# rssalessio/TZDDPC

Hardware: AMD Instinct MI355X
Metric: MPC steps/sec (batched trajectories), double-integrator N=20 (higher is better)
Workload: dtype f64

## Files before the change

### tzddpc_amd/csrc/tz_ipm.hip.h

```cpp
#pragma once

#define TZ_MINWAVES 4
#define TZ_RLEV_CARRY_MAX 2
#define TZ_RLEV_GATE 1e6
#define TZ_SEED_VIOL_MAX 0.1

struct TzEll { int L, VL; const TzEllEnt* ent; const int* seg; const double* val; const unsigned short* idx; };
typedef __attribute__((address_space(1))) const char* tz_gptr;
typedef __attribute__((address_space(1))) const tz_d2* tz_gd2ptr;
__device__ inline double tz_ell_walk(const char* base_, unsigned lo, int L, unsigned stride, const double* in) {
  double a0 = 0.0, a1 = 0.0;
  const char* b = reinterpret_cast<const char*>(in);
  tz_gptr base = (tz_gptr)base_;
  int e = 0;
  for (; e + 3 < L; e += 4) {
    tz_gptr q0 = base, q1 = base + stride, q2 = base + 2 * (size_t)stride, q3 = base + 3 * (size_t)stride;
    asm volatile("" : "+s"(q0), "+s"(q1), "+s"(q2), "+s"(q3));
    const tz_d2 r0 = *(tz_gd2ptr)(q0 + lo), r1 = *(tz_gd2ptr)(q1 + lo), r2 = *(tz_gd2ptr)(q2 + lo), r3 = *(tz_gd2ptr)(q3 + lo);
    base += 4 * (size_t)stride;
    a0 += r0.x * *reinterpret_cast<const double*>(b + tz_ell_off(r0.y));
    a1 += r1.x * *reinterpret_cast<const double*>(b + tz_ell_off(r1.y));
    a0 += r2.x * *reinterpret_cast<const double*>(b + tz_ell_off(r2.y));
    a1 += r3.x * *reinterpret_cast<const double*>(b + tz_ell_off(r3.y));
  }
// ... 418 lines not shown
    }
    if (pacc) { unsigned long long t1 = __builtin_amdgcn_s_memtime(); pacc[hh == 0 ? PH_GRAM_RED : PH_GRAM_RMW] += t1 - tq0; tq0 = t1; }
    if (hh == 0) __syncthreads();
    if (pacc && hh == 0) { unsigned long long t1 = __builtin_amdgcn_s_memtime(); pacc[PH_GRAM_BAR] += t1 - tq0; tq0 = t1; }
  }
}

__device__ inline void tz_form_H_ksplit(const IpmParams& p, double* Hq, const double* Pq, const double* wv, const int* sm, unsigned long long* pacc) {
  const int wave = __builtin_amdgcn_readfirstlane(threadIdx.x >> 6);
  const int g = wave >> 1, h = wave & 1;
  if (p.Tz > 7) { if (g == 0) tz_gram_rows<0, 7>(p, Hq, Pq, wv, sm, h, pacc); else tz_gram_rows<7, 10>(p, Hq, Pq, wv, sm, h, pacc); }
  else          { if (g == 0) tz_gram_rows<0, 5>(p, Hq, Pq, wv, sm, h, pacc); else tz_gram_rows<5, 7>(p, Hq, Pq, wv, sm, h, pacc); }
}

__device__ inline void tz_gram(const IpmParams& p, double* Hq, const double* Pq, const double* wv, const int* kl, unsigned long long* pacc = nullptr) {
  if (p.ksplit) tz_form_H_ksplit(p, Hq, Pq, wv, kl, pacc);
  else tz_form_H(p, Hq, wv, kl);
}

__device__ inline void tz_sqrt_rsqrt(double d, double& sq, double& rs) {
  double y = __builtin_amdgcn_rsq(d);
  double g = d * y, h = 0.5 * y;
  double r = __builtin_fma(-h, g, 0.5);
  g = __builtin_fma(g, r, g); h = __builtin_fma(h, r, h);
  const double e = __builtin_fma(-g, g, d);
  g = __builtin_fma(e, h, g);
  double inv = h + h;
  const double e2 = __builtin_fma(-g, inv, 1.0);
  inv = __builtin_fma(e2, inv, inv);
  sq = g; rs = inv;
}

__device__ inline double tz_recip(double x) {
  double y = __builtin_amdgcn_rcp(x);
  y = __builtin_fma(__builtin_fma(-x, y, 1.0), y, y);
  y = __builtin_fma(__builtin_fma(-x, y, 1.0), y, y);
  return y;
}

template <int JJ>
__device__ inline double tz_quad_bcast(double v) {
  const unsigned long long u = __builtin_bit_cast(unsigned long long, v);
  constexpr int ctrl = JJ * 0x55;
  const unsigned lo = (unsigned)__builtin_amdgcn_mov_dpp((int)(unsigned)u, ctrl, 0xf, 0xf, true);
  const unsigned hi = (unsigned)__builtin_amdgcn_mov_dpp((int)(unsigned)(u >> 32), ctrl, 0xf, 0xf, true);
  return __builtin_bit_cast(double, ((unsigned long long)hi << 32) | lo);
}

__device__ inline void tz_factor_col(int Tz, double* Hq, double* dinv, int* flag, int pp, int tid, int nthr) {
  const int dbase = (tz_qprefix(pp) + (pp >> 2)) * TZ_QSTR + 4 * (pp & 3);
  const double a00 = Hq[dbase], a10 = Hq[dbase + TZ_QROW], a11 = Hq[dbase + TZ_QROW + 1];
  const double a20 = Hq[dbase + 2 * TZ_QROW], a21 = Hq[dbase + 2 * TZ_QROW + 1], a22 = Hq[dbase + 2 * TZ_QROW + 2];
  const double a30 = Hq[dbase + 3 * TZ_QROW], a31 = Hq[dbase + 3 * TZ_QROW + 1], a32 = Hq[dbase + 3 * TZ_QROW + 2], a33 = Hq[dbase + 3 * TZ_QROW + 3];
  bool ok = true;
  double l00, i00, l11, i11, l22, i22, l33, i33;
  ok = ok && (a00 > 0.0);
  tz_sqrt_rsqrt(fmax(a00, 1e-300), l00, i00);
  const double l10 = a10 * i00, l20 = a20 * i00, l30 = a30 * i00;
  const double d1 = a11 - l10 * l10; ok = ok && (d1 > 0.0);
  tz_sqrt_rsqrt(fmax(d1, 1e-300), l11, i11);
  const double l21 = (a21 - l20 * l10) * i11, l31 = (a31 - l30 * l10) * i11;
  const double d2 = a22 - l20 * l20 - l21 * l21; ok = ok && (d2 > 0.0);
  tz_sqrt_rsqrt(fmax(d2, 1e-300), l22, i22);
  const double l32 = (a32 - l30 * l20 - l31 * l21) * i22;
  const double d3 = a33 - l30 * l30 - l31 * l31 - l32 * l32; ok = ok && (d3 > 0.0);
  tz_sqrt_rsqrt(fmax(d3, 1e-300), l33, i33);
  (void)l00; (void)l11; (void)l22; (void)l33;
  {
    const double m10 = -l10 * i00 * i11;
    const double m21 = -l21 * i11 * i22;
    const double m32 = -l32 * i22 * i33;
    const double m20 = -(l20 * i00 + l21 * m10) * i22;
    const double m31 = -(l31 * i11 + l32 * m21) * i33;
    const double m30 = -(l30 * i00 + l31 * m10 + l32 * m20) * i33;
    if (tid == 0 && !ok) *flag = 1;
    if (tid == 0) {
      double* m = dinv + pp * 16;
      m[0] = i00;
      m[4] = m10; m[5] = i11;
      m[8] = m20; m[9] = m21; m[10] = i22;
      m[12] = m30; m[13] = m31; m[14] = m32; m[15] = i33;
    }
  }
  for (int t = tid; t < 4 * (Tz - pp - 1); t += nthr) {
    const int I = pp + 1 + (t >> 2), i = t & 3;
    const int base = (tz_qprefix(I) + (pp >> 2)) * TZ_QSTR + TZ_QROW * i + 4 * (pp & 3);
    const double b0 = Hq[base], b1 = Hq[base + 1], b2 = Hq[base + 2], b3 = Hq[base + 3];
    const double x0 = b0 * i00;
    const double x1 = (b1 - x0 * l10) * i11;
    const double x2 = (b2 - x0 * l20 - x1 * l21) * i22;
    const double x3 = (b3 - x0 * l30 - x1 * l31 - x2 * l32) * i33;
    Hq[base] = x0; Hq[base + 1] = x1; Hq[base + 2] = x2; Hq[base + 3] = x3;
  }
}

__device__ inline void tz_wave_sync() {
  __builtin_amdgcn_fence(__ATOMIC_RELEASE, "wavefront");
  __builtin_amdgcn_wave_barrier();
  __builtin_amdgcn_fence(__ATOMIC_ACQUIRE, "wavefront");
}
__device__ inline bool tz_spin_until(const int* f, int target) {
  for (int guard = 0; guard < (1 << 20); ++guard) {
    const int v = __builtin_amdgcn_readfirstlane(__hip_atomic_load(f, __ATOMIC_ACQUIRE, __HIP_MEMORY_SCOPE_WORKGROUP));
    if (v >= target) return true;
    __builtin_amdgcn_s_sleep(1);
  }
  return false;
}

__device__ inline void tz_cholesky_wave(const IpmParams& p, double* Hq, double* dinv, int* flag, int* prog = nullptr) {
  const int Tz = p.Tz;
  const int lane = tz_tid() & 63;
  const int k = lane >> 4, blk = (lane >> 2) & 3, ij = lane & 3;
  for (int pp = 0; pp < Tz; ++pp) {
    if (pp > 0) {
      const int pq = pp >> 2, po = 4 * (pp & 3);
      const double* pb = Hq + tz_qprefix(pp) * TZ_QSTR + TZ_QROW * ij + k;
      for (int g = 0; pp + 4 * g < Tz; g += 2) {
        const int Ia = pp + 4 * g + blk, Ib = Ia + 4;
        const bool va = Ia < Tz, vb = Ib < Tz;
        const int qa = tz_qprefix(va ? Ia : pp), qb = tz_qprefix(vb ? Ib : pp);
        const double* pa = Hq + qa * TZ_QSTR + TZ_QROW * ij + k;
        const double* pa2 = Hq + qb * TZ_QSTR + TZ_QROW * ij + k;
        double* pc = Hq + (qa + pq) * TZ_QSTR + TZ_QROW * k + po + ij;
        double* pc2 = Hq + (qb + pq) * TZ_QSTR + TZ_QROW * k + po + ij;
        double a0 = *pc, a1 = 0.0, c0 = vb ? *pc2 : 0.0, c1 = 0.0;
        int off = 0, k2 = 0;
        for (; k2 + 1 < pp; k2 += 2) {
          const int off1 = off + 4 + (((k2 & 3) == 3) ? TZ_QSTR - 16 : 0);
          const double nb0 = -pb[off], nb1 = -pb[off1];
          const double x0 = pa[off], x1 = pa[off1], y0 = pa2[off], y1 = pa2[off1];
          a0 = __builtin_amdgcn_mfma_f64_4x4x4f64(x0, nb0, a0, 0, 0, 0);
          c0 = __builtin_amdgcn_mfma_f64_4x4x4f64(y0, nb0, c0, 0, 0, 0);
          a1 = __builtin_amdgcn_mfma_f64_4x4x4f64(x1, nb1, a1, 0, 0, 0);
          c1 = __builtin_amdgcn_mfma_f64_4x4x4f64(y1, nb1, c1, 0, 0, 0);
          off = off1 + 4 + ((((k2 + 1) & 3) == 3) ? TZ_QSTR - 16 : 0);
        }
        if (k2 < pp) {
          const double nb0 = -pb[off];
          a0 = __builtin_amdgcn_mfma_f64_4x4x4f64(pa[off], nb0, a0, 0, 0, 0);
          c0 = __builtin_amdgcn_mfma_f64_4x4x4f64(pa2[off], nb0, c0, 0, 0, 0);
        }
        if (va) *pc = a0 + a1;
        if (vb) *pc2 = c0 + c1;
      }
      tz_wave_sync();
    }
    tz_factor_col(Tz, Hq, dinv, flag, pp, lane, 64);
    tz_wave_sync();
    if (prog && lane == 0) __hip_atomic_store(prog, pp + 1, __ATOMIC_RELEASE, __HIP_MEMORY_SCOPE_WORKGROUP);
  }
}

__device__ inline void tz_chol_solve_wave(const IpmParams& p, const double* Hq, const double* dinv, const double* rhs, double* out, bool bwd_only = false) {
  const int tt = tz_tid();
  if (tt >= 64) return;
  __builtin_amdgcn_s_setprio(TZ_PRIO_SOLVE);
  const int Tz = p.Tz, nzp = p.nzp;
  const int t = tt, jq = t & 3, tq = t >> 2;
  double rv = (t < nzp) ? rhs[t] : 0.0;
  const int rowbase = tz_qprefix(tq < Tz ? tq : 0) * TZ_QSTR + TZ_QROW * jq;
  auto fwd_load = [&](int I, double (&mm)[4], double (&ll)[4]) {
    const int Ic = I < Tz ? I : Tz - 1;
    const double* m = dinv + Ic * 16 + 4 * jq;
    const int base = rowbase + (Ic >> 2) * TZ_QSTR + 4 * (Ic & 3);
    const bool below = tq > Ic && tq < Tz;
#pragma unroll
    for (int k = 0; k < 4; ++k) { mm[k] = m[k]; ll[k] = below ? Hq[base + k] : 0.0; }
  };
  double mA[4], lA[4], mB[4], lB[4];
  auto fwd_step = [&](int I, const double (&mm)[4], const double (&ll)[4]) {
    const double a0 = tz_quad_bcast<0>(rv), a1 = tz_quad_bcast<1>(rv), a2 = tz_quad_bcast<2>(rv), a3 = tz_quad_bcast<3>(rv);
    const double yc = (mm[0] * a0 + mm[1] * a1) + (mm[2] * a2 + mm[3] * a3);
    const double y0 = tz_readlane(yc, 4 * I), y1 = tz_readlane(yc, 4 * I + 1), y2 = tz_readlane(yc, 4 * I + 2), y3 = tz_readlane(yc, 4 * I + 3);
    rv = (tq == I) ? yc : rv - ((ll[0] * y0 + ll[1] * y1) + (ll[2] * y2 + ll[3] * y3));
  };
  if (!bwd_only) {
  fwd_load(0, mA, lA);
  for (int I = 0; I < Tz; I += 2) {
    fwd_load(I + 1, mB, lB);
    fwd_step(I, mA, lA);
    fwd_load(I + 2, mA, lA);
    if (I + 1 < Tz) fwd_step(I + 1, mB, lB);
  }
  }
  const int colbase = (t >> 4) * TZ_QSTR + 4 * ((t >> 2) & 3) + (t & 3);
  auto bwd_load = [&](int I, double (&mm)[4], double (&ll)[4]) {
    const int Ic = I >= 0 ? I : 0;
    const double* m = dinv + Ic * 16 + jq;
    const int base = tz_qprefix(Ic) * TZ_QSTR + colbase;
    const bool above = tq < Ic;
#pragma unroll
    for (int k = 0; k < 4; ++k) { mm[k] = m[4 * k]; ll[k] = above ? Hq[base + k * TZ_QROW] : 0.0; }
  };
  bwd_load(Tz - 1, mA, lA);
  for (int I = Tz - 1; I >= 0; I -= 2) {
    bwd_load(I - 1, mB, lB);
    fwd_step(I, mA, lA);
    bwd_load(I - 2, mA, lA);
    if (I - 1 >= 0) fwd_step(I - 1, mB, lB);
  }
  if (t < nzp) out[t] = rv;
  __builtin_amdgcn_s_setprio(0);
}

__device__ inline bool tz_fwd_trailing(const IpmParams& p, const double* Hq, const double* dinv, double rv, const int* prog, double* yout) {
  const int Tz = p.Tz, nzp = p.nzp;
  const int t = tz_tid() & 63, jq = t & 3, tq = t >> 2;
  const int rowbase = tz_qprefix(tq < Tz ? tq : 0) * TZ_QSTR + TZ_QROW * jq;
  bool ok = true;
  for (int I = 0; I < Tz; ++I) {
    if (!tz_spin_until(prog, I + 1)) { ok = false; break; }
    const double* m = dinv + I * 16 + 4 * jq;
    const int base = rowbase + (I >> 2) * TZ_QSTR + 4 * (I & 3);
    const bool below = tq > I && tq < Tz;
    double mm[4], ll[4];
#pragma unroll
    for (int k = 0; k < 4; ++k) { mm[k] = m[k]; ll[k] = below ? Hq[base + k] : 0.0; }
    const double a0 = tz_quad_bcast<0>(rv), a1 = tz_quad_bcast<1>(rv), a2 = tz_quad_bcast<2>(rv), a3 = tz_quad_bcast<3>(rv);
    const double yc = (mm[0] * a0 + mm[1] * a1) + (mm[2] * a2 + mm[3] * a3);
    const double y0 = tz_readlane(yc, 4 * I), y1 = tz_readlane(yc, 4 * I + 1), y2 = tz_readlane(yc, 4 * I + 2), y3 = tz_readlane(yc, 4 * I + 3);
    rv = (tq == I) ? yc : rv - ((ll[0] * y0 + ll[1] * y1) + (ll[2] * y2 + ll[3] * y3));
  }
  if (t < nzp) yout[t] = rv;
  return ok;
}

#include "tz_tt.hip.h"
#define TZ_TT_NST 4
#define TZ_TT_AFTER_CHOL(p, H, dinv) do { tz_tt_block_inverse(p, H, dinv); __syncthreads(); } while (0)
#define TZ_TT_SOLVE(p, H, dinv, rhs, ybuf, out) tz_chol_solve_blk(p, H, rhs, ybuf, out)


typedef __attribute__((address_space(4))) const IpmParams* TzKargPtr;

template <int MAXR, int NCG, int MINW = TZ_MINWAVES>
__global__ __launch_bounds__(TZ_THREADS, MINW) void tz_ipm_kernel(IpmParams p) {
#if TZ_PROFILE
  const bool PROF = p.prof != nullptr && blockIdx.x == 0;
#else
  constexpr bool PROF = false;
#endif
  unsigned long long tprev = 0, tstart = 0;
  unsigned long long acc_ph[PH_COUNT] = {};
#define TZ_STAMP(ph) do { if (PROF) { unsigned long long _t = __builtin_amdgcn_s_memtime(); acc_ph[ph] += _t - tprev; tprev = _t; } } while (0)
  if (PROF) { tprev = __builtin_amdgcn_s_memtime(); tstart = tprev; }
  extern __shared__ double lds[];
  const int b = blockIdx.x;
  int t = threadIdx.x;
#define TZ_FRESH_T() asm volatile("" : "+v"(t))
#define TZ_COLS(c, lim) if (const int c = t; c < (lim))
  const bool wave0 = __builtin_amdgcn_readfirstlane(threadIdx.x >> 6) == 0;
  const bool wave1 = __builtin_amdgcn_readfirstlane(threadIdx.x >> 6) == 1;
  const int nz = p.nz, mi = p.mi, nzp = p.nzp, mip = p.mip;
  const FuseParams& F0 = p.F;
  const bool fused = F0.on != 0;
  if (!fused && p.prestatus[b] != 0) {
    if (t == 0) { p.status[b] = 3; p.iters[b] = 0; if (p.status_copy) p.status_copy[b] = 3; }
    TZ_COLS(c, nz) p.x[(size_t)b * nz + c] = 0.0;
    for (int r = t; r < mi; r += TZ_THREADS) { p.s[(size_t)b * mi + r] = 1.0; p.lam[(size_t)b * mi + r] = 0.0; }
    return;
  }
  constexpr bool TT = (NCG >= 2);
  const size_t hsize = TT ? (size_t)p.ntile * p.TS : (size_t)p.nquads * TZ_QSTR;
  double* Hq = lds;
  double* dinv = Hq + hsize;
  double* dfac = dinv + p.Tz * 16;
  double* xv = dfac + (TT ? 16 : 0);
  double* dxv = xv + nzp;
  double* rdv = dxv + nzp;
  double* r1v = rdv + nzp;
  double* qv = r1v + nzp;
  double* tmpz = qv + nzp;
  double* part = tmpz + nzp;
  double* part2 = part + 4 * nzp;
  double* vin = part2 + 4 * nzp;
  double* red = vin + mip + 4;
  int* flag = (int*)(red + 32);
  int* kl = (int*)(red + 34);
  double* thl = red + 34 + (p.nklist + 1) / 2;
  double* stl = thl + p.F.ntheta;
  double* pl = stl + 4 * TZ_NMAX;
  double* tbl = pl + p.nell;
  double* Pq = tbl + p.ntube;
  constexpr bool PARK = (MINW == 4);
  double* hL = Pq + (p.ksplit ? hsize : 0);
  double* gL = hL + mip;

  double s_[MAXR], l_[MAXR], h_[MAXR], gx_[MAXR];
#define TZ_H(k, r) (PARK ? hL[r] : h_[k])
#define TZ_GX(k, r) (PARK ? gL[r] : gx_[k])
#define TZ_SET_H(k, r, v) do { if (PARK) hL[r] = (v); else h_[k] = (v); } while (0)
#define TZ_ADD_GX(k, r, v) do { if (PARK) gL[r] += (v); else gx_[k] += (v); } while (0)
#define TZ_ROWS(k, r) _Pragma("unroll") for (int k = 0; k < MAXR; ++k) if (const int r = t + TZ_THREADS * k; r < mi)
  int rseg_[MAXR];
#pragma unroll
  for (int k = 0; k < MAXR; ++k) { const int r = t + TZ_THREADS * k; rseg_[k] = (r < mi) ? p.eg.seg[r] : 0; }
  const int ccol = (nzp <= 64 && t >= 64) ? (t < 128 ? t - 64 : nz) : t;
  const int cseg = (ccol < nz) ? p.et.seg[ccol] : 0;

  if (TT) { (void)kl; (void)Pq; }
  else if (p.ksplit) {
    for (int i = t; i <= ((p.Kc + 3) >> 2); i += TZ_THREADS) kl[i] = p.smask[i];
    for (int e = t; e < p.nquads * 64; e += TZ_THREADS) {
      const int qd = e >> 6;
      int I = 0;
      while (tz_qprefix(I + 1) <= qd) ++I;
      const int r = 4 * I + ((e >> 4) & 3), c = 4 * (4 * (qd - tz_qprefix(I)) + ((e >> 2) & 3)) + (e & 3);
      double v = (c < nzp) ? p.P[(size_t)r * nzp + c] : 0.0;
      if (r == c) v = (r < nz) ? v + p.reg : 1.0;
      Pq[qd * TZ_QSTR + TZ_QROW * ((e >> 4) & 3) + (e & 15)] = v;
    }
  }
  else for (int i = t; i < p.nklist; i += TZ_THREADS) kl[i] = p.klist[i];
  if (fused) {
    const int n = F0.fin.n, m = F0.fin.m, nv = F0.fin.N * m;
    const int n1 = (F0.tube.pmax + 1) * n * n, n2 = n1 + (F0.tube.pmax > 0 ? F0.tube.pmax : 1) * (n + m) * n;
    for (int i = t; i < n2; i += TZ_THREADS) tbl[i] = (i < n1) ? F0.tube.CKpow[i] : F0.tube.T[i - n1];
    double* ec = tbl + n2;
    const double* plA = F0.plant.A + (size_t)b * F0.plant.A_stride;
    const double* plB = F0.plant.Bm + (size_t)b * F0.plant.B_stride;
    for (int i = t; i < n * n; i += TZ_THREADS) { ec[i] = plA[i]; ec[2 * n * m + n * n + n + i] = F0.fin.R2[i]; ec[2 * n * m + 2 * n * n + n + i] = F0.fin.Phi[(size_t)n * n + i]; }
    for (int i = t; i < n * m; i += TZ_THREADS) { ec[n * n + i] = plB[i]; ec[n * n + n * m + i] = F0.plant.K[i]; }
    for (int i = t; i < n; i += TZ_THREADS) ec[n * n + 2 * n * m + i] = F0.fin.r1[i];
    for (int i = t; i < n * nv; i += TZ_THREADS) ec[3 * n * n + 2 * n * m + n + i] = F0.fin.Gam[(size_t)n * nv + i];
    for (int i = t; i < nv; i += TZ_THREADS) ec[3 * n * n + 2 * n * m + n + n * nv + i] = F0.fin.Dz[i];
    int* pwl = (int*)(ec + 3 * n * n + 2 * n * m + n + n * nv + nv);
    for (int i = t; i < F0.fin.N; i += TZ_THREADS) pwl[i] = F0.tube.power[i];
  }
  if (fused && t < F0.fin.n) {
    stl[t] = F0.plant.x[(size_t)b * F0.fin.n + t];
    stl[F0.fin.n + t] = F0.plant.xbar[(size_t)b * F0.fin.n + t];
    stl[2 * F0.fin.n + t] = F0.plant.e[(size_t)b * F0.fin.n + t];
  }
#pragma unroll
  for (int k = 0; k < MAXR; ++k) { s_[k] = 1.0; l_[k] = 0.0; h_[k] = 0.0; gx_[k] = 0.0; }
  TZ_COLS(c, nzp) xv[c] = 0.0;
  for (int c = t; c < p.Tz * 16; c += TZ_THREADS) dinv[c] = 0.0;
  for (int r = t; r < mip + 4; r += TZ_THREADS) vin[r] = 0.0;
  __syncthreads();

  const int nsteps = fused ? F0.nsteps : 1;
  if (fused && F0.sticky_fresh != 0 && t == 0 && F0.plant.sticky) F0.plant.sticky[b] = 0;
  int was_shifted = (p.warm != 0 && (p.shift_policy >= 2 || p.shift_state[b] == -2)) ? p.shift_state[b] : 0;
  int status = 1, it = 0;
  int work_f = 0, work_s = 0;
  int rlev_carry = 0;
  unsigned brk_hi = 0;
  int rpar = 0;
  for (int step = 0; step < nsteps; ++step) {
  TZ_FRESH_T();
  TzKargPtr kp0 = (TzKargPtr)__builtin_amdgcn_kernarg_segment_ptr();
  asm volatile("" : "+s"(kp0));
  const FuseParams& F = ((const IpmParams*)kp0)->F;
  const IpmParams& pk = *(const IpmParams*)kp0;
  int src = 0;
  if (step == 0) src = (pk.warm != 0 && pk.prev_status != nullptr && pk.prev_status[b] == 0) ? 1 : 0;
  else src = (pk.warm_steps != 0 && status == 0) ? 2 : 0;
  bool skip = false;
  double wpre = 0.0;
  if (fused && t < F.fin.n) wpre = F.plant.w[(size_t)b * F.plant.w_stride + (size_t)step * F.w_step + t];
  bool shifted = false;
  const bool seeded = src != 0 && was_shifted == -2;
  if (seeded) {
    was_shifted = (pk.shift_policy >= 2) ? 1 : 0;
  } else if (src != 0) {
    const int prev_it = (step == 0) ? pk.iters[b] : it;
    const bool quiet_run = was_shifted > 0 && prev_it <= 1;
    const int nquiet = quiet_run ? was_shifted : 0;
    const bool back = was_shifted < 0 && prev_it >= 1;
    shifted = pk.shift_policy == 1 || (pk.shift_policy >= 2 && (prev_it >= pk.shift_policy || back || (quiet_run && (pk.shift_quiet == 0 || nquiet <= pk.shift_quiet))));
    was_shifted = shifted ? 1 + nquiet : (((quiet_run && pk.shift_policy >= 2) || (was_shifted < 0 && !back)) ? -1 : 0);
  }
  const bool inlaunch = fused && src == 2;
  const bool walk_early = inlaunch && (shifted || (step & 7) == 0);
  if (fused) {
    if (t == 0) { flag[0] = 0; flag[1] = 0; }
    const int n = F.fin.n, m = F.fin.m, nv = F.fin.N * m;
// ... 56 lines not shown
      }
      __syncthreads();
      e1 = red[14];
    } else {
      if (t < nzp) rdv[t] = (t < nz) ? (tz_ell_colsum(pl, cseg) + qv[t]) + part[t] : 0.0;
      __syncthreads();
      double e2 = 0, e3 = 0;
      TZ_COLS(c, nz) e1 = fmax(e1, fabs(rdv[c]));
      tz_block_reduce3<RED_MAX, RED_MAX, RED_MAX, 1>(e1, e2, e3, red, rpar);
    }
    TZ_STAMP(PH_RD_C);
    return e1;
  };

  int attempt = 0;
retry_solve:
  const bool retried = attempt != 0;
  bool okf = true;
  bool warm = !skip && src != 0;
  double scq = 0, sch = 0;
  if (!skip) {
  if (warm) {
    if (src == 1) {
      if (shifted) {
        TZ_COLS(c, nz) xv[c] = pk.x[(size_t)b * nz + pk.sx[c]] * pk.sxs[c];
        TZ_ROWS(k, r) l_[k] = pk.lam[(size_t)b * mi + pk.sr[r]] * pk.sls[r];
      } else {
        TZ_COLS(c, nz) xv[c] = pk.x[(size_t)b * nz + c];
        TZ_ROWS(k, r) l_[k] = pk.lam[(size_t)b * mi + r];
      }
    }
    if (walk_early && !retried) { tz_ell_gemv_sum<MAXR>(pl, rseg_, gx_); if (PARK) { TZ_ROWS(k, r) gL[r] = gx_[k]; } }
    else if (src != 2 || retried) { tz_ell_gemv<MAXR, TT>(p, xv, pl, rseg_, gx_); if (PARK) { TZ_ROWS(k, r) gL[r] = gx_[k]; } }
    TZ_STAMP(PH_WARM_A);
    double viol = 0.0;
    TZ_ROWS(k, r) { const double hv = TZ_H(k, r); viol = fmax(viol, TZ_GX(k, r) - hv); sch = fmax(sch, fabs(hv)); }
    TZ_COLS(c, nz) scq = fmax(scq, fabs(qv[c]));
    tz_block_reduce3<RED_MAXU, RED_MAXU, RED_MAXU>(viol, scq, sch, red, rpar);
    TZ_STAMP(PH_WARM_B);
    if (seeded && viol > TZ_SEED_VIOL_MAX) { warm = false; TZ_ROWS(k, r) l_[k] = 1.0; }
    else {
    const double sig = fmin(fmax(pk.warm_floor, pk.warm_gain * viol), pk.warm_cap);
    const double sig2 = sig * sig;
    TZ_ROWS(k, r) {
      s_[k] = fmax(TZ_H(k, r) - TZ_GX(k, r), sig);
      l_[k] = fmax(l_[k], sig2 * tz_recip(s_[k]));
      vin[r] = l_[k];
    }
    }
  }
  if (!warm) {
    was_shifted = 0;
    TZ_ROWS(k, r) vin[r] = 1.0;
    __syncthreads();
    if constexpr (TT) tz_gram_tt<TZ_TT_GU(MINW), TZ_TT_NST>(p, Hq, vin); else tz_gram(p, Hq, Pq, vin, kl);
    __syncthreads();
    TZ_ROWS(k, r) vin[r] = TZ_H(k, r);
    __syncthreads();
    if (!wave0) tz_ell_gemvT_part<TT>(p, vin, pl);
    __syncthreads();
    if (t < nzp) r1v[t] = (t < nz) ? tz_ell_colsum(pl, cseg) - qv[t] : 0.0;
    __syncthreads();
    if constexpr (TT) { okf = tz_cholesky_tt(p, Hq, dinv, dfac, flag); TZ_TT_AFTER_CHOL(p, Hq, dinv); TZ_TT_SOLVE(p, Hq, dinv, r1v, tmpz, xv); }
    else {
    if (wave0) tz_cholesky_wave(p, Hq, dinv, flag);
    __syncthreads(); okf = (*flag == 0);
    tz_chol_solve_wave(p, Hq, dinv, r1v, xv);
    }
    tz_ell_gemv<MAXR, TT>(p, xv, pl, rseg_, gx_);
    if (PARK) { TZ_ROWS(k, r) gL[r] = gx_[k]; }
  }
  if (!warm) {
    double rmin = 1e300;
    scq = 0.0; sch = 0.0;
    TZ_ROWS(k, r) { const double hv = TZ_H(k, r); rmin = fmin(rmin, hv - TZ_GX(k, r)); sch = fmax(sch, fabs(hv)); }
    TZ_COLS(c, nz) scq = fmax(scq, fabs(qv[c]));
    tz_block_reduce3<RED_MIN, RED_MAX, RED_MAX>(rmin, scq, sch, red, rpar);
    const double shift = (rmin <= 1e-8) ? fmax(0.0, 1.0 - rmin) : 0.0;
    TZ_ROWS(k, r) s_[k] = TZ_H(k, r) - TZ_GX(k, r) + shift;
  }
  }
  red[12] = 1.0 + scq; red[13] = 1.0 + sch;

  status = skip ? 3 : (okf ? 1 : 2);
  TZ_STAMP(PH_WARM);
  bool px_in_part = false;
  int rlev = retried ? 2 : 0;
  unsigned brk_now = 0;
  __builtin_amdgcn_s_setprio(0);
  for (it = 0; it < pk.max_iter && status == 1; ++it) {
    __builtin_amdgcn_s_setprio(TZ_PRIO_ELEM);
    TZ_FRESH_T();
    TzKargPtr kpi = (TzKargPtr)__builtin_amdgcn_kernarg_segment_ptr();
    asm volatile("" : "+s"(kpi));
    const IpmParams& pi = *(const IpmParams*)kpi;
    TZ_STAMP(PH_STEP);
    double w_[MAXR], rp_[MAXR], ds_[MAXR], dl_[MAXR], g_[MAXR], is_[MAXR], il_[MAXR];
#pragma unroll
    for (int k = 0; k < MAXR; ++k) { w_[k] = 0.0; rp_[k] = 0.0; ds_[k] = 0.0; dl_[k] = 0.0; g_[k] = 0.0; is_[k] = 1.0; il_[k] = 1.0; }
    double nrp = 0, sl = 0, z0 = 0;
    TZ_ROWS(k, r) { rp_[k] = TZ_GX(k, r) + s_[k] - TZ_H(k, r); nrp = fmax(nrp, fabs(rp_[k])); sl += s_[k] * l_[k]; }
    TZ_STAMP(PH_T1);
    tz_block_reduce3<RED_MAXU, RED_SUM, RED_SUM, 2>(nrp, sl, z0, red, rpar);
    TZ_STAMP(PH_T2);
    const double mu = sl * pi.inv_mi;
    nrp *= tz_recip(red[13]);
    if (!(mu == mu) || !(nrp == nrp) || mu > 1e200) { status = 2; break; }
    TZ_STAMP(PH_T3);
    const bool fresh_warm = (it == 0) && warm;
    if ((nrp <= pi.tol_res && mu <= pi.mu_tol) || (mu <= pi.mu_floor && !fresh_warm)) {
      const double e1 = exact_rd(fresh_warm);
      const double nrd = e1 * tz_recip(red[12]);
      TZ_STAMP(PH_GEMVT);
      if (!(nrd == nrd)) { status = 2; break; }
      if (nrd <= pi.tol_res && nrp <= pi.tol_res && mu <= pi.mu_tol) { status = 0; px_in_part = true; break; }
      if (mu <= pi.mu_floor && !fresh_warm) { status = (nrd <= pi.tol_loose && nrp <= pi.tol_loose) ? 0 : 2; px_in_part = true; break; }
    }
    TZ_ROWS(k, r) { is_[k] = tz_recip(s_[k]); il_[k] = tz_recip(l_[k]); w_[k] = l_[k] * is_[k]; vin[r] = w_[k]; }
    __syncthreads();
    TZ_STAMP(PH_TOP);
    if constexpr (TT) {
      if (rlev == 0 && rlev_carry != 0 && warm && (unsigned)__builtin_amdgcn_readfirstlane((int)tz_hi(mu)) <= brk_hi)
        rlev = rlev_carry < TZ_RLEV_CARRY_MAX ? rlev_carry : TZ_RLEV_CARRY_MAX;
    }
    bool okc;
    __builtin_amdgcn_s_setprio(0);
    if constexpr (TT) tz_gram_tt<TZ_TT_GU(MINW), TZ_TT_NST>(p, Hq, vin, (PROF && t == 0) ? acc_ph : nullptr); else tz_gram(p, Hq, Pq, vin, kl, (PROF && t == 0) ? acc_ph : nullptr);
    __syncthreads();
    TZ_STAMP(PH_FORM);
    TZ_FRESH_T();
    if (rlev != 0) {
      const double rx = (rlev == 1) ? 1e-9 : (rlev == 2) ? 1e-6 : (rlev == 3) ? 1e-3 : 1.0;
      TZ_COLS(c, nz) {
        const int I = c >> 2, i = c & 3;
        Hq[TT ? (size_t)(((I * (I + 1)) >> 1) + I) * p.TS + 5 * i : (size_t)tz_hidx(c, c)] += rx;
      }
    }
    TZ_ROWS(k, r) vin[r] = w_[k] * rp_[k];
    if (t == 0) { flag[2] = 0; flag[3] = 0; }
    __syncthreads();
    if constexpr (!TT) {
      if (wave0) {
        __builtin_amdgcn_s_setprio(TZ_PRIO);
        tz_cholesky_wave(p, Hq, dinv, flag, flag + 2);
        __builtin_amdgcn_s_setprio(0);
      } else {
        tz_ell_gemvT_part<TT>(p, vin, pl);
        tz_gemvT_partial<NCG, 1, 3>(p.P, p.nP, nzp, xv, part2);
        tz_wave_sync();
        if ((tz_tid() & 63) == 0) __hip_atomic_fetch_add(flag + 3, 1, __ATOMIC_RELEASE, __HIP_MEMORY_SCOPE_WORKGROUP);
        if (wave1) {
          bool ok1 = tz_spin_until(flag + 3, 3);
          const int c = tz_tid() & 63;
          double rv = 0.0;
          if (c < nzp) {
            const double pxq = (c < nz) ? tz_gemvT_get3(part2, nzp, c) + qv[c] : 0.0;
            rdv[c] = pxq;
            rv = (c < nz) ? -pxq - tz_ell_colsum(pl, cseg) : 0.0;
          }
          ok1 = tz_fwd_trailing(p, Hq, dinv, rv, flag + 2, tmpz) && ok1;
          if (!ok1 && c == 0) flag[0] = 3;
        }
      }
      __syncthreads();
      okc = (*flag == 0);
      TZ_STAMP(PH_CHOL);
    } else {
      if (wave0) tz_gemvT_partial<NCG, 0, 1>(p.P, p.nP, nzp, xv, part2);
      else tz_ell_gemvT_part<TT>(p, vin, pl);
      __syncthreads();
      TZ_COLS(c, nzp) {
        const double pxq = (c < nz) ? part2[c] + qv[c] : 0.0;
        rdv[c] = pxq;
        r1v[c] = (c < nz) ? -pxq - tz_ell_colsum(pl, cseg) : 0.0;
      }
      __syncthreads();
      TZ_STAMP(PH_GEMVT);
      okc = tz_cholesky_tt(p, Hq, dinv, dfac, flag, (PROF && t == 0) ? acc_ph : nullptr);
      TZ_TT_AFTER_CHOL(p, Hq, dinv);
      TZ_STAMP(PH_CHOL);
    }
    if (!okc) {
      if (rlev >= 4) { status = 2; break; }
      if constexpr (TT) { if (brk_now == 0) brk_now = (unsigned)__builtin_amdgcn_readfirstlane((int)tz_hi(mu * TZ_RLEV_GATE)); }
      rlev = __builtin_amdgcn_readfirstlane(rlev + 1);
      __syncthreads();
      if (t == 0) flag[0] = 0;
      __syncthreads();
      continue;
    }
    TZ_FRESH_T();
    if constexpr (TT) TZ_TT_SOLVE(p, Hq, dinv, r1v, tmpz, dxv);
    else tz_chol_solve_wave(p, Hq, dinv, tmpz, dxv, true);
    __syncthreads();
    TZ_STAMP(PH_SOLVE);
    tz_ell_gemv<MAXR, TT>(p, dxv, pl, rseg_, g_);
    TZ_STAMP(PH_GEMV);
    __builtin_amdgcn_s_setprio(TZ_PRIO_ELEM);
    TZ_FRESH_T();
    double mp = 0.0, md = 0.0, z4 = 0;
    TZ_ROWS(k, r) {
      const double ds = -rp_[k] - g_[k];
      const double dl = -l_[k] - w_[k] * ds;
      ds_[k] = ds; dl_[k] = dl;
      mp = fmax(mp, -ds * is_[k]);
      md = fmax(md, -dl * il_[k]);
      z4 += (s_[k] + ds) * (l_[k] + dl);
    }
    tz_block_reduce3<RED_MAXU, RED_MAXU, RED_SUM>(mp, md, z4, red, rpar);
    const double ap = tz_recip(fmax(1.0, mp)), ad = tz_recip(fmax(1.0, md));
    double muaff = z4;
    if (mp > 1.0 || md > 1.0) {
      double z1 = 0, z2 = 0;
      muaff = 0.0;
      TZ_ROWS(k, r) muaff += (s_[k] + ap * ds_[k]) * (l_[k] + ad * dl_[k]);
      tz_block_reduce3<RED_SUM, RED_SUM, RED_SUM, 1>(muaff, z1, z2, red, rpar);
    }
    muaff *= pi.inv_mi;
    const double sfr = (attempt == 0) ? pi.step_frac : pi.step_frac_retry;
    if (fmin(ap, ad) >= pi.aff_thr && muaff <= pi.aff_mu * mu) {
      const double mmA = fmax(mp, md);
      const double alphaA = (mmA > sfr) ? sfr * tz_recip(mmA) : 1.0;
      TZ_COLS(c, nz) xv[c] += alphaA * dxv[c];
      TZ_ROWS(k, r) { s_[k] += alphaA * ds_[k]; l_[k] += alphaA * dl_[k]; TZ_ADD_GX(k, r, alphaA * g_[k]); }
      __syncthreads();
      continue;
    }
    double sigma = muaff * tz_recip(mu); sigma = sigma * sigma * sigma;
    TZ_FRESH_T();
    TZ_ROWS(k, r) {
      const double rc = s_[k] * l_[k] + ds_[k] * dl_[k] - sigma * mu;
      vin[r] = l_[k] + (l_[k] * rp_[k] - rc) * is_[k];
      ds_[k] = rc;
    }
    __syncthreads();
    TZ_STAMP(PH_ELEM);
    __builtin_amdgcn_s_setprio(0);
    if (!wave0) tz_ell_gemvT_part<TT>(p, vin, pl);
    __syncthreads();
    TZ_COLS(c, nzp) r1v[c] = (c < nz) ? -rdv[c] - tz_ell_colsum(pl, cseg) : 0.0;
    __syncthreads();
    TZ_STAMP(PH_GEMVT);
    if constexpr (TT) TZ_TT_SOLVE(p, Hq, dinv, r1v, tmpz, dxv);
    else tz_chol_solve_wave(p, Hq, dinv, r1v, dxv);
    __syncthreads();
    TZ_STAMP(PH_SOLVE);
    tz_ell_gemv<MAXR, TT>(p, dxv, pl, rseg_, g_);
    TZ_STAMP(PH_GEMV);
    __builtin_amdgcn_s_setprio(TZ_PRIO_ELEM);
    double ms = 0.0, ml = 0.0, z3 = 0;
    TZ_ROWS(k, r) {
      const double rc = ds_[k];
      const double ds = -rp_[k] - g_[k];
      const double dl = (-rc - l_[k] * ds) * is_[k];
      ds_[k] = ds; dl_[k] = dl;
      ms = fmax(ms, -ds * is_[k]);
      ml = fmax(ml, -dl * il_[k]);
    }
    tz_block_reduce3<RED_MAXU, RED_MAXU, RED_SUM, 2>(ms, ml, z3, red, rpar);
    const double mm = fmax(ms, ml);
    const double alpha = (mm * 1.0 > sfr) ? sfr * tz_recip(mm) : 1.0;
    TZ_COLS(c, nz) xv[c] += alpha * dxv[c];
    TZ_ROWS(k, r) { s_[k] += alpha * ds_[k]; l_[k] += alpha * dl_[k]; TZ_ADD_GX(k, r, alpha * g_[k]); }
    __syncthreads();
  }
  __builtin_amdgcn_s_setprio(TZ_PRIO_GLUE);
  TZ_FRESH_T();
  work_f = __builtin_amdgcn_readfirstlane(work_f + it + ((warm || skip) ? 0 : 1));
  if (TT && status == 0 && !skip && attempt == 0) {
    if (brk_now != 0) { rlev_carry = __builtin_amdgcn_readfirstlane(rlev); brk_hi = brk_now; }
    else if (rlev == 0) { rlev_carry = 0; brk_hi = 0; }
  }
  if (status != 0 && !skip && attempt == 0) {
    attempt = 1; src = 0;
    __syncthreads();
    if (t == 0) flag[0] = 0;
    TZ_COLS(c, nzp) xv[c] = 0.0;
    TZ_ROWS(k, r) { s_[k] = 1.0; l_[k] = 1.0; }
    __syncthreads();
    goto retry_solve;
  }
  if (status != 0 && !skip) {
    double lm = 0.0, z1 = 0.0, z2 = 0.0;
    TZ_ROWS(k, r) lm = fmax(lm, l_[k]);
    tz_block_reduce3<RED_MAX, RED_MAX, RED_MAX, 1>(lm, z1, z2, red, rpar);
    const bool lm_ok = lm > 0.0 && lm < 1e300;
    const double il = lm_ok ? 1.0 / lm : 0.0;
    double hy = 0.0;
    TZ_ROWS(k, r) { const double y = lm_ok ? l_[k] * il : 0.0; vin[r] = y; hy += TZ_H(k, r) * y; }
    __syncthreads();
    if (!wave0) tz_ell_gemvT_part<TT>(p, vin, pl);
    __syncthreads();
    double gmax = fabs(tz_ell_colsum(pl, cseg));
    tz_block_reduce3<RED_MAX, RED_SUM, RED_SUM, 2>(gmax, hy, z2, red, rpar);
    if (lm_ok && hy < -1e-6 && gmax <= 1e-6 * fmax(1.0, -hy)) status = 3;
    TZ_COLS(c, nzp) xv[c] = 0.0;
    px_in_part = false;
    __syncthreads();
  }
  work_s += 1;
  TzKargPtr kpe = (TzKargPtr)__builtin_amdgcn_kernarg_segment_ptr();
  asm volatile("" : "+s"(kpe));
  const IpmParams& pe = *(const IpmParams*)kpe;
  if (step == nsteps - 1) {
    TZ_COLS(c, nz) pe.x[(size_t)b * nz + c] = xv[c];
    TZ_ROWS(k, r) { pe.s[(size_t)b * mi + r] = s_[k]; pe.lam[(size_t)b * mi + r] = l_[k]; }
    if (t == 0) {
      pe.status[b] = status; pe.iters[b] = it;
      pe.shift_state[b] = was_shifted;
      if (pe.status_copy) pe.status_copy[b] = status;
      if (pe.work) { atomicAdd(pe.work, (unsigned long long)work_f); atomicAdd(pe.work + 1, (unsigned long long)work_s); atomicMax(pe.work + 2, (unsigned long long)work_f); }
    }
  }
  TZ_STAMP(PH_ELEM);
  if (fused) {
    TzKargPtr kp1 = (TzKargPtr)__builtin_amdgcn_kernarg_segment_ptr();
    asm volatile("" : "+s"(kp1));
    const FuseParams& F = ((const IpmParams*)kp1)->F;
    const int n = F.fin.n, m = F.fin.m, N = F.fin.N, nv = N * m;
    const double* x0 = stl + n;
    const double* ec = tbl + (F.tube.pmax + 1) * n * n + (F.tube.pmax > 0 ? F.tube.pmax : 1) * (n + m) * n;
    const double *cA = ec, *cB = ec + n * n, *cK = cB + n * m, *cr1 = cK + n * m, *cR2 = cr1 + n, *cPhi = cR2 + n * n, *cGam = cPhi + n * n, *cDz = cGam + n * nv;
    const bool want_cost = F.cost_step != 0 || step == nsteps - 1;
    if (F.lean_epilogue != 0 && !want_cost && !F.fin.v && !F.fin.xbar) {
      if (skip) __syncthreads();
      if (t == 0 && status != 0 && F.plant.sticky && F.plant.sticky[b] == 0) F.plant.sticky[b] = status;
      if (t < 64) {
        const PlantParams& Q = F.plant;
        double xn = 0.0, xb = 0.0;
        if (t < n) {
          xn = stl[3 * TZ_NMAX + t];
          for (int j = 0; j < n; ++j) { xn += cA[t * n + j] * stl[j]; xb += cPhi[t * n + j] * x0[j]; }
          for (int j = 0; j < m; ++j) {
            const double v0 = cDz[j] * xv[F.fin.vpos ? F.fin.vpos[j] : j];
            double u = v0;
            for (int i = 0; i < n; ++i) u += cK[j * n + i] * stl[2 * n + i];
            xn += cB[t * m + j] * u; xb += cGam[t * nv + j] * v0;
            if (t == 0 && Q.u_out) Q.u_out[(size_t)b * Q.u_stride + (size_t)step * F.u_step + j] = u;
          }
        }
        __builtin_amdgcn_fence(__ATOMIC_RELEASE, "wavefront");
        __builtin_amdgcn_wave_barrier();
        __builtin_amdgcn_fence(__ATOMIC_ACQUIRE, "wavefront");
        if (t < n) {
          stl[t] = xn; stl[n + t] = xb; stl[2 * n + t] = xn - xb;
          if (Q.x_out) Q.x_out[(size_t)b * Q.x_stride + (size_t)step * F.x_step + t] = xn;
        }
      }
      __syncthreads();
      TZ_STAMP(PH_EPILOGUE);
      continue;
    }
    __syncthreads();
    if (want_cost && !px_in_part) tz_gemvT_partial<NCG>(p.P, p.nP, nzp, xv, part);
    if (F.fin.recy) {
      for (int c = t; c < nv; c += TZ_THREADS) {
        double a = F.fin.rec0[c];
        for (int j = 0; j < n; ++j) a += F.fin.recx[(size_t)c * n + j] * x0[j];
        for (int k = 0; k < nz; ++k) a += F.fin.recy[(size_t)c * nz + k] * xv[k];
        dxv[c] = a;
      }
    } else
    for (int c = t; c < nv; c += TZ_THREADS) dxv[c] = cDz[c] * xv[F.fin.vpos ? F.fin.vpos[c] : c];
    __syncthreads();
    TZ_STAMP(PH_EPI_A);
    double acc = 0.0, z1 = 0.0, z2 = 0.0;
    if (want_cost) {
      TZ_COLS(c, nz) acc += xv[c] * (0.5 * (px_in_part ? part[c] : tz_gemvT_get(part, nzp, c)) + qv[c]);
      tz_block_reduce3<RED_SUM, RED_SUM, RED_SUM, 1>(acc, z1, z2, red, rpar);
    }
    if (t == 0 && !want_cost) { if (status != 0 && F.plant.sticky && F.plant.sticky[b] == 0) F.plant.sticky[b] = status; }
    if (t == 0 && want_cost) {
      double r = F.fin.r0;
      for (int i = 0; i < n; ++i) {
        r += cr1[i] * x0[i];
        for (int j = 0; j < n; ++j) r += x0[i] * cR2[i * n + j] * x0[j];
      }
      F.fin.cost[(size_t)b * F.fin.cost_stride + (size_t)step * F.cost_step] = (status == 0) ? acc / F.fin.cost_scale + r : INFINITY;
      if (status != 0 && F.plant.sticky && F.plant.sticky[b] == 0) F.plant.sticky[b] = status;
    }
    if (F.fin.v) for (int c = t; c < nv; c += TZ_THREADS) F.fin.v[(size_t)b * nv + c] = dxv[c];
    if (F.fin.xbar) {
      for (int r = t; r < (N + 1) * n; r += TZ_THREADS) {
        double a = 0.0;
        for (int j = 0; j < n; ++j) a += F.fin.Phi[(size_t)r * n + j] * x0[j];
        const double* g = F.fin.Gam + (size_t)r * nv;
        for (int c = 0; c < nv; ++c) a += g[c] * dxv[c];
        F.fin.xbar[(size_t)b * (N + 1) * n + r] = a;
      }
    }
    {
      const int ln = t & 63;
      for (int i = __builtin_amdgcn_readfirstlane(t >> 6); i < n; i += TZ_NWAVES) {
        double a = (ln < n) ? cPhi[i * n + ln] * x0[ln] : 0.0;
        for (int c = ln; c < nv; c += 64) a += cGam[i * nv + c] * dxv[c];
        a = tz_wave_reduce<RED_SUM>(a);
        if (ln == 0) tmpz[i] = a;
// ... 42 lines not shown
```

Baseline: 101.6 million.

## Replace triangular solves with explicit block-inverse of Cholesky factor via MFMA

While wave0 factors the matrix, wave1 now builds the explicit inverse of the lower-triangular Cholesky factor in place using f64 MFMA, replacing the trailing forward substitution. Both per-iteration solves then become two parallel matrix-vector products spread across the block, with a DPP reduction instead of serial wave-level substitution. This removes the sequential dependency chain of the triangular solves. The cost is extra inverse computation overlapped with factorization, possible numerical differences from forming the explicit inverse, and in-place overwriting of Hq.

```diff
diff --git a/tzddpc_amd/csrc/tz_ipm.hip.h b/tzddpc_amd/csrc/tz_ipm.hip.h
--- a/tzddpc_amd/csrc/tz_ipm.hip.h
+++ b/tzddpc_amd/csrc/tz_ipm.hip.h
@@ -594,7 +594,7 @@
   }
 }
 
-__device__ inline void tz_chol_solve_wave(const IpmParams& p, const double* Hq, const double* dinv, const double* rhs, double* out, bool bwd_only = false) {
+__device__ inline void tz_chol_solve_wave(const IpmParams& p, const double* Hq, const double* dinv, const double* rhs, double* out) {
   const int tt = tz_tid();
   if (tt >= 64) return;
   __builtin_amdgcn_s_setprio(TZ_PRIO_SOLVE);
@@ -617,14 +617,12 @@
     const double y0 = tz_readlane(yc, 4 * I), y1 = tz_readlane(yc, 4 * I + 1), y2 = tz_readlane(yc, 4 * I + 2), y3 = tz_readlane(yc, 4 * I + 3);
     rv = (tq == I) ? yc : rv - ((ll[0] * y0 + ll[1] * y1) + (ll[2] * y2 + ll[3] * y3));
   };
-  if (!bwd_only) {
   fwd_load(0, mA, lA);
   for (int I = 0; I < Tz; I += 2) {
     fwd_load(I + 1, mB, lB);
     fwd_step(I, mA, lA);
     fwd_load(I + 2, mA, lA);
     if (I + 1 < Tz) fwd_step(I + 1, mB, lB);
-  }
   }
   const int colbase = (t >> 4) * TZ_QSTR + 4 * ((t >> 2) & 3) + (t & 3);
   auto bwd_load = [&](int I, double (&mm)[4], double (&ll)[4]) {
@@ -646,26 +644,82 @@
   __builtin_amdgcn_s_setprio(0);
 }
 
-__device__ inline bool tz_fwd_trailing(const IpmParams& p, const double* Hq, const double* dinv, double rv, const int* prog, double* yout) {
-  const int Tz = p.Tz, nzp = p.nzp;
-  const int t = tz_tid() & 63, jq = t & 3, tq = t >> 2;
-  const int rowbase = tz_qprefix(tq < Tz ? tq : 0) * TZ_QSTR + TZ_QROW * jq;
-  bool ok = true;
-  for (int I = 0; I < Tz; ++I) {
-    if (!tz_spin_until(prog, I + 1)) { ok = false; break; }
-    const double* m = dinv + I * 16 + 4 * jq;
-    const int base = rowbase + (I >> 2) * TZ_QSTR + 4 * (I & 3);
-    const bool below = tq > I && tq < Tz;
-    double mm[4], ll[4];
-#pragma unroll
-    for (int k = 0; k < 4; ++k) { mm[k] = m[k]; ll[k] = below ? Hq[base + k] : 0.0; }
-    const double a0 = tz_quad_bcast<0>(rv), a1 = tz_quad_bcast<1>(rv), a2 = tz_quad_bcast<2>(rv), a3 = tz_quad_bcast<3>(rv);
-    const double yc = (mm[0] * a0 + mm[1] * a1) + (mm[2] * a2 + mm[3] * a3);
-    const double y0 = tz_readlane(yc, 4 * I), y1 = tz_readlane(yc, 4 * I + 1), y2 = tz_readlane(yc, 4 * I + 2), y3 = tz_readlane(yc, 4 * I + 3);
-    rv = (tq == I) ? yc : rv - ((ll[0] * y0 + ll[1] * y1) + (ll[2] * y2 + ll[3] * y3));
-  }
-  if (t < nzp) yout[t] = rv;
-  return ok;
+__device__ inline bool tz_inverse_trailing(const IpmParams& p, double* Hq, const double* dinv, const int* prog) {
+  const int Tz = p.Tz;
+  const int lane = tz_tid() & 63;
+  const int k = lane >> 4, blk = (lane >> 2) & 3, ij = lane & 3;
+  const int aoff = TZ_QROW * ij + k;
+  const int boff = TZ_QROW * k + (lane & 15);
+  for (int I = 1; I < Tz; ++I) {
+    if (!tz_spin_until(prog, I)) return false;
+    const int qI = tz_qprefix(I);
+    double acc0 = 0.0, acc1 = 0.0, acc2 = 0.0, acc3 = 0.0;
+    for (int K = 0; K < I; ++K) {
+      const double a = Hq[(qI + (K >> 2)) * TZ_QSTR + 4 * (K & 3) + aoff];
+      const double* xk = Hq + tz_qprefix(K) * TZ_QSTR + boff;
+      const double mk = dinv[K * 16 + 4 * k + ij];
+#define TZ_INV_STEP(g, acc) if (4 * (g) <= K) { \
+        const int J = 4 * (g) + blk; \
+        const double xv_ = (J < K) ? xk[(g) * TZ_QSTR] : mk; \
+        acc = __builtin_amdgcn_mfma_f64_4x4x4f64(a, (J <= K) ? xv_ : 0.0, acc, 0, 0, 0); }
+      TZ_INV_STEP(0, acc0) TZ_INV_STEP(1, acc1) TZ_INV_STEP(2, acc2) TZ_INV_STEP(3, acc3)
+#undef TZ_INV_STEP
+    }
+    if (!tz_spin_until(prog, I + 1)) return false;
+    const double nm = -dinv[I * 16 + 4 * ij + k];
+    const int ng = ((I - 1) >> 2) + 1;
+    const double x0 = __builtin_amdgcn_mfma_f64_4x4x4f64(nm, acc0, 0.0, 0, 0, 0);
+    const double x1 = (ng > 1) ? __builtin_amdgcn_mfma_f64_4x4x4f64(nm, acc1, 0.0, 0, 0, 0) : 0.0;
+    const double x2 = (ng > 2) ? __builtin_amdgcn_mfma_f64_4x4x4f64(nm, acc2, 0.0, 0, 0, 0) : 0.0;
+    const double x3 = (ng > 3) ? __builtin_amdgcn_mfma_f64_4x4x4f64(nm, acc3, 0.0, 0, 0, 0) : 0.0;
+    double* xo = Hq + qI * TZ_QSTR + boff;
+    if (blk < I) xo[0] = x0;
+    if (4 + blk < I) xo[TZ_QSTR] = x1;
+    if (8 + blk < I) xo[2 * TZ_QSTR] = x2;
+    if (12 + blk < I) xo[3 * TZ_QSTR] = x3;
+    tz_wave_sync();
+  }
+  return true;
+}
+
+__device__ inline void tz_inv_solve(const IpmParams& p, const double* Hq, const double* dinv, const double* rhs, double* ybuf, double* out) {
+  const int tt = tz_tid();
+  const int Tz = p.Tz;
+  const int r = tt >> 2, g = tt & 3, I = r >> 2, i = r & 3;
+  const bool live = I < Tz;
+  __builtin_amdgcn_s_setprio(TZ_PRIO_SOLVE);
+  double acc = 0.0;
+  if (live) {
+    const double* xr = Hq + (tz_qprefix(I) + g) * TZ_QSTR + TZ_QROW * i;
+    const double* mr = dinv + I * 16 + 4 * i;
+#pragma unroll
+    for (int jt = 0; jt < 4; ++jt) {
+      const int J = 4 * g + jt;
+      if (J <= I) {
+        const double* s = (J < I) ? xr + 4 * jt : mr;
+        const double* v = rhs + 4 * J;
+        acc += (s[0] * v[0] + s[1] * v[1]) + (s[2] * v[2] + s[3] * v[3]);
+      }
+    }
+  }
+  acc += tz_dpp_mov<0xB1>(acc);
+  acc += tz_dpp_mov<0x4E>(acc);
+  if (live && g == 0) ybuf[r] = acc;
+  __syncthreads();
+  acc = 0.0;
+  if (live) {
+    for (int I2 = I + g; I2 < Tz; I2 += 4) {
+      const bool diag = I2 == I;
+      const double* s = diag ? dinv + I * 16 + i : Hq + (tz_qprefix(I2) + (I >> 2)) * TZ_QSTR + 4 * (I & 3) + i;
+      const int str = diag ? 4 : TZ_QROW;
+      const double* v = ybuf + 4 * I2;
+      acc += (s[0] * v[0] + s[str] * v[1]) + (s[2 * str] * v[2] + s[3 * str] * v[3]);
+    }
+  }
+  acc += tz_dpp_mov<0xB1>(acc);
+  acc += tz_dpp_mov<0x4E>(acc);
+  if (live && g == 0) out[r] = acc;
+  __builtin_amdgcn_s_setprio(0);
 }
 
 #include "tz_tt.hip.h"
@@ -1028,13 +1082,12 @@
         if (wave1) {
           bool ok1 = tz_spin_until(flag + 3, 3);
           const int c = tz_tid() & 63;
-          double rv = 0.0;
           if (c < nzp) {
             const double pxq = (c < nz) ? tz_gemvT_get3(part2, nzp, c) + qv[c] : 0.0;
             rdv[c] = pxq;
-            rv = (c < nz) ? -pxq - tz_ell_colsum(pl, cseg) : 0.0;
+            r1v[c] = (c < nz) ? -pxq - tz_ell_colsum(pl, cseg) : 0.0;
           }
-          ok1 = tz_fwd_trailing(p, Hq, dinv, rv, flag + 2, tmpz) && ok1;
+          ok1 = tz_inverse_trailing(p, Hq, dinv, flag + 2) && ok1;
           if (!ok1 && c == 0) flag[0] = 3;
         }
       }
@@ -1067,7 +1120,7 @@
     }
     TZ_FRESH_T();
     if constexpr (TT) TZ_TT_SOLVE(p, Hq, dinv, r1v, tmpz, dxv);
-    else tz_chol_solve_wave(p, Hq, dinv, tmpz, dxv, true);
+    else tz_inv_solve(p, Hq, dinv, r1v, part2, dxv);
     __syncthreads();
     TZ_STAMP(PH_SOLVE);
     tz_ell_gemv<MAXR, TT>(p, dxv, pl, rseg_, g_);
@@ -1118,7 +1171,7 @@
     __syncthreads();
     TZ_STAMP(PH_GEMVT);
     if constexpr (TT) TZ_TT_SOLVE(p, Hq, dinv, r1v, tmpz, dxv);
-    else tz_chol_solve_wave(p, Hq, dinv, r1v, dxv);
+    else tz_inv_solve(p, Hq, dinv, r1v, part2, dxv);
     __syncthreads();
     TZ_STAMP(PH_SOLVE);
     tz_ell_gemv<MAXR, TT>(p, dxv, pl, rseg_, g_);
```

Measured after the change: 101.2 million. No clear change (-0.4%).
